# UbiquityRobotics/fiducials

Measured on AMD Instinct MI355X. Metric: frames/sec @1920x1080 20-marker (aruco detect + pose hot path), higher is better.
Workload: dtype u8

## Files before the change

### fiducials_amd/csrc/fid_api.hip

```cpp
#include "fid_kernels.hip"

#include <math.h>
#include <stdio.h>
#include <stdlib.h>
#include <string.h>

#include <new>
#include <string>
#include <vector>

namespace {

enum { ST_GRAY = 0, ST_THRESH, ST_STARTS, ST_PROBE, ST_WALK, ST_APPROX, ST_SORT, ST_NEAR, ST_RESOLVE, ST_IDENT, ST_FILTER, ST_SUBPIX, ST_POSE, ST_SEEDWALK,
       ST_SEEDLESS, ST_COUNT };
const char *const kStageNames[ST_COUNT] = {"to_gray", "threshold", "find_starts", "walk_probe", "walk_full", "approx", "sort_cands",
                                           "near", "resolve", "identify", "filter_markers", "subpix", "pose", "seed_walk", "seedless_chain"};
enum { EV_SEEDWALK0 = 14, EV_SEEDWALK1, EV_SEEDLESS0, EV_SEEDLESS1, EV_POSE0, EV_POSE1, EV_COUNT };
static_assert(EV_SEEDWALK0 > ST_SUBPIX + 1, "the brackets lie behind the stage boundaries");

constexpr int TX = 128, TY = 32, NT = 256;
constexpr int THRW_NT = 512, THRW_WT = 16;
static_assert(THRW_NT * THRW_WT >= 8191, "k_threshold_wide: a row per workgroup");

}

struct fid_ctx;

struct PoseAsk {
    fid_camera cam;
    double len;
    bool cov;
    double sigma;
    fid_map_robust_opts opts;
};

struct PoseRequest {
    enum Kind { MARKER, MAP, MAP_ROBUST };
    Kind kind;
    PoseAsk ask = {};
    bool armed = false;
    bool at_hand = false;
    explicit PoseRequest(Kind k) : kind(k) {}
    inline bool ahead(const fid_ctx *c) const;
    void forget() { at_hand = false; }
    void finished(const fid_ctx *c) { at_hand = ahead(c); }
    bool answers(const PoseAsk &a) const
    {
        return at_hand && !memcmp(&ask.cam, &a.cam, sizeof a.cam) && ask.len == a.len && ask.opts.inlier_px == a.opts.inlier_px &&
               ask.opts.min_markers == a.opts.min_markers && (!a.cov || (ask.cov && ask.sigma == a.sigma));
    }
    void answered(const PoseAsk &a)
    {
        ask = a;
        armed = at_hand = getenv("FID_NO_POSE_AHEAD") == nullptr;
    }
};

struct fid_ctx {
    int device = 0;
    hipStream_t stream = nullptr;
    enum { MAX_SUB = 8 };
    struct Tuning {
        int sub_frames = 0;
        bool sub_shares_set = false;
        int sub_share[MAX_SUB] = {64, 36}, n_sub_share = 2;
        int feed_share[4] = {20, 30, 30, 20};
        int pieces = 0;
        int stagger = 0;
        int fs_barrier = 0;
        int chain_at = 0;
        bool idx_stream = true;
        bool prio = false;
        int thr_xcd = 1;
        int thr_nw = 3, thr_split = 0, thr_rows = 0;
        int seed_shift = 0;
        int seed_kernel = 0;
        bool trace_legacy = false;
        int walk_blocks = 0;
        int walk_blocks_cap = 0;
        int walk2_div = 6;
        int sw_blocks = 0;
        int copy_blocks = 0;
        int probe_refill = 4;
        int probe_refill0 = 0;
        int probe_passes = 1;
        int probe_single = 16;
        int segc_warm = 1;
        int light_x = 1;
        int resolve_lds_kb = 64;
        int resolve_serial = 0;
        int resolve_reg_max = 64;
        int tail_grid = 4096;
        int filter_lds = 256;
    } tune;
    hipStream_t sub_stream[MAX_SUB] = {};
    int sub_prio[MAX_SUB] = {};
    hipStream_t aux_stream[MAX_SUB] = {};
    hipStream_t idx_stream = nullptr;
    hipEvent_t aux_fork[MAX_SUB] = {}, aux_join[MAX_SUB] = {}, aux_idx[MAX_SUB] = {};
    hipEvent_t sub_done[MAX_SUB] = {}, fork_ev = nullptr;
    hipStream_t copy_stream = nullptr;
    hipEvent_t in_ready[MAX_SUB] = {};
    hipEvent_t tail_ev = nullptr, wait_ev = nullptr;
    hipEvent_t wait_copy_ev = nullptr;
    hipEvent_t fs_done[MAX_SUB] = {};
    hipEvent_t walk_done[MAX_SUB] = {};
    hipEvent_t front_done[MAX_SUB] = {};
    hipEvent_t sub_ev[MAX_SUB][EV_COUNT] = {};
    bool blocking = false;
    bool chained = false;
    bool host_feed = false;
    bool from_host_call = false;
    bool piece_chain = false;
    bool tail_recorded = false;
    bool whole_border_walk = false;
    struct Pending {
        const uint8_t *d_src;
        int F, W, H, stride;
        long long fstride;
        fid_encoding enc;
    } pend = {};
    bool in_flight = false;
    bool fed_from_host = false;
    fid_params params;
    fid_limits lim;
    DevParams P;
    std::vector<uint8_t> dict_host;
// ... 106 lines not shown
}

bool refuse_in_flight(fid_ctx *c)
{
    if (c->in_flight) c->last_error = "a submitted batch is in flight: fid_collect first";
    return c->in_flight;
}
bool refuse_no_map(fid_ctx *c)
{
    if (c->map_n == 0) c->last_error = "no map: fid_set_map first";
    return c->map_n == 0;
}
bool refuse_room(fid_ctx *c, int cap_frames)
{
    if (cap_frames < c->last_frames)
        c->last_error = "caller room for " + std::to_string(cap_frames) + " frames, the last call had " + std::to_string(c->last_frames);
    return cap_frames < c->last_frames;
}

int roundup(int v, int m) { return (v + m - 1) / m * m; }

size_t results_bytes(int F, int MM)
{
    auto up = [](size_t v) { return (v + 255) & ~(size_t)255; };
    return up(sizeof(DevGlobal)) + up(sizeof(unsigned) * fid_ctx::MAX_SUB) + up(sizeof(DevCounts) * (size_t)F) + up(sizeof(fid_marker) * (size_t)F * MM) +
           up(sizeof(fid_pose_out) * (size_t)F * MM);
}
void layout_results(fid_ctx *c, int F)
{
    auto up = [](size_t v) { return (v + 255) & ~(size_t)255; };
    const int MM = c->lim.max_markers_per_frame;
    size_t off = 0;
    c->d_global = (DevGlobal *)(c->d_res + off);
    c->h_global = (DevGlobal *)(c->h_res + off);
    off += up(sizeof(DevGlobal));
    c->d_nwork = (unsigned *)(c->d_res + off);
    off += up(sizeof(unsigned) * fid_ctx::MAX_SUB);
    c->d_counts = (DevCounts *)(c->d_res + off);
    c->h_counts = (DevCounts *)(c->h_res + off);
    off += up(sizeof(DevCounts) * (size_t)F);
    c->res_clear_bytes = off;
    c->d_markers = (fid_marker *)(c->d_res + off);
    c->h_markers = (fid_marker *)(c->h_res + off);
    off += up(sizeof(fid_marker) * (size_t)F * MM);
    c->res_markers_end = off;
    c->res_poses_off = off;
    c->d_poses = (fid_pose_out *)(c->d_res + off);
    c->h_poses = (fid_pose_out *)(c->h_res + off);
    off += up(sizeof(fid_pose_out) * (size_t)F * MM);
    c->res_poses_end = off;
}

template <int NW, bool SPLIT>
void launch_thr_stream(dim3 grid, hipStream_t st, const uint8_t *g, long long gfstride, uint32_t *masks, const DevParams &P, int RS, int xcd_map)
{
    using S = ThrStream<3, 4, 13, NW>;
    fid_launch_log("k_threshold_stream", S::NT, S::LDS_BYTES);
    k_threshold_stream<3, 4, 13, NW, SPLIT><<<grid, dim3(S::NT), S::LDS_BYTES, st>>>(g, gfstride, masks, P, RS, xcd_map);
}

fid_status apply_params(fid_ctx *c, const fid_params *p)
{
    if (p->adaptiveThreshWinSizeMin < 3 || p->adaptiveThreshWinSizeMax < p->adaptiveThreshWinSizeMin ||
        p->adaptiveThreshWinSizeStep <= 0)
        return FID_E_INVALID_ARG;
    if (!(p->minMarkerPerimeterRate > 0 && p->maxMarkerPerimeterRate > 0 && p->polygonalApproxAccuracyRate > 0 &&
          p->minCornerDistanceRate >= 0 && p->minDistanceToBorder >= 0 && p->minMarkerDistanceRate >= 0))
        return FID_E_INVALID_ARG;
    if (p->markerBorderBits <= 0) return FID_E_INVALID_ARG;
    int nsc = (p->adaptiveThreshWinSizeMax - p->adaptiveThreshWinSizeMin) / p->adaptiveThreshWinSizeStep + 1;
    if (nsc > FID_MAX_SCALES) return FID_E_UNSUPPORTED;
    DevParams &P = c->P;
    P.nscales = nsc;
    P.rmax = 0;
    for (int i = 0; i < nsc; i++) {
        long long w = p->adaptiveThreshWinSizeMin + (long long)i * p->adaptiveThreshWinSizeStep;
        if (w % 2 == 0) w++;
        if (w > FID_MAX_THR_WIN) {
            c->last_error = "adaptive threshold window " + std::to_string(w) + " px: windows above " + std::to_string(FID_MAX_THR_WIN) +
                            " px (2 x 8191 + 1) are not supported";
            return FID_E_UNSUPPORTED;
        }
        P.win[i] = (int)w;
        if (w / 2 > P.rmax) P.rmax = (int)(w / 2);
    }
    {
        double cdelta = p->adaptiveThreshConstant;
        int i = (int)cdelta;
        P.idelta = i - (i > cdelta);
    }
    P.polyAcc = p->polygonalApproxAccuracyRate;
    P.minCornerDistRate = p->minCornerDistanceRate;
    P.minMarkerDistRate = p->minMarkerDistanceRate;
    P.minDistToBorder = p->minDistanceToBorder;
    P.markerSize = c->dict_ms;
    P.borderBits = p->markerBorderBits;
    P.cellSize = p->perspectiveRemovePixelPerCell;
    P.cellMargin = (int)(p->perspectiveRemoveIgnoredMarginPerCell * p->perspectiveRemovePixelPerCell);
    if (P.markerSize + 2 * P.borderBits > FID_MAX_CELLS) {
        c->last_error = "markerSize + 2 x markerBorderBits = " + std::to_string(P.markerSize + 2 * P.borderBits) + " cells: at most " +
                        std::to_string(FID_MAX_CELLS) + " are supported";
        return FID_E_UNSUPPORTED;
    }
    if (P.cellSize < 1 || P.cellSize - 2 * P.cellMargin < 1) return FID_E_UNSUPPORTED;
    if ((long long)(P.markerSize + 2 * P.borderBits) * P.cellSize > FID_MAX_PATCH) {
        c->last_error = "unwarped patch of (markerSize + 2 x markerBorderBits) x perspectiveRemovePixelPerCell = " +
                        std::to_string((long long)(P.markerSize + 2 * P.borderBits) * P.cellSize) + " px a side: at most " +
                        std::to_string(FID_MAX_PATCH) + " are supported";
        return FID_E_UNSUPPORTED;
    }
    P.minOtsuStdDev = p->minOtsuStdDev;
// ... 210 lines not shown
inline T *frames_from(T *base, int f0, size_t per_frame)
{
    return base ? base + (size_t)f0 * per_frame : nullptr;
}

SubBatch sub_batch_view(fid_ctx *c, const SubPlan &plan, int sb, const uint8_t *d_src, long long fstride, const uint8_t *gray, long long gfstride, int W,
                        int H)
{
    SubBatch s;
    s.sb = sb;
    s.nsub = plan.nsub;
    s.f0 = plan.f0[sb];
    s.Fs = plan.f0[sb + 1] - s.f0;
    s.P = c->P;
    s.P.nframes = s.Fs;
    const DevParams &P = s.P;
    const int f0 = s.f0, lane = c->piece_chain ? (sb & 1) : sb;
    s.st = s.nsub > 1 ? c->sub_stream[lane] : c->stream;
    s.sa = c->aux_stream[lane];
    s.si = (s.nsub == 1 && s.Fs <= 16 && c->idx_stream) ? c->idx_stream : s.sa;
    s.tail = c->piece_chain ? s.sa : s.st;
    s.ev = c->sub_ev[sb];
    const size_t MC = (size_t)P.maxCands, MM = (size_t)P.maxMarkers, MCn = (size_t)P.maxContours, msb = (size_t)(P.markerSize + 2 * P.borderBits);
    s.src = d_src + (long long)f0 * fstride;
    s.gray_dst = c->d_gray + (size_t)f0 * W * H;
    s.g = gray + (long long)f0 * gfstride;
    s.gfstride = gfstride;
    const size_t MS = (size_t)P.maxStarts, chunks = (size_t)P.maxChunks;
    s.masks = frames_from(c->d_masks, f0, (size_t)P.nscales * P.TR * P.TC * MT_ROWS);
    s.starts = frames_from(c->d_starts, f0, MS), s.surv1 = frames_from(c->d_surv1, f0, MS), s.surv = frames_from(c->d_surv, f0, MS);
    s.contours = frames_from(c->d_contours, f0, MCn);
    s.tab = frames_from(c->d_ckpts, f0, 2 * MCn * chunk_tab_pitch(P)), s.pool = frames_from(c->d_pool, f0, chunks * CKW);
    s.counts = c->d_counts + f0;
    s.seedq = frames_from(c->d_seedq, f0, MCn), s.segs = frames_from(c->d_segs, f0, MCn), s.pend = frames_from(c->d_pend, f0, MCn);
    s.seedhash = frames_from(c->d_seedhash, f0, (size_t)P.seedHashCap);
    s.wres = frames_from(c->d_wres, f0, MCn), s.cinfo = frames_from(c->d_cinfo, f0, MCn), s.recs = frames_from(c->d_recs, f0, 2 * MCn);
    s.cbase = frames_from(c->d_cbase, f0, MCn), s.dense = frames_from(c->d_dense, f0, chunks * (CK / 4));
    s.cands = frames_from(c->d_cands, f0, MC), s.sorted = frames_from(c->d_sorted, f0, MC), s.filtered = frames_from(c->d_filtered, f0, MC);
    s.cmeta = frames_from(c->d_cmeta, f0, MC), s.nearb = frames_from(c->d_near, f0, MC * (MC / 32));
    s.worklist = frames_from(c->d_worklist, f0, MC), s.nwork = c->d_nwork + sb;
    s.ident = frames_from(c->d_ident, f0, MC), s.bits = frames_from(c->d_bits, f0, MC * msb * msb);
    s.pre = frames_from(c->d_pre, f0, MM), s.markers = frames_from(c->d_markers, f0, MM), s.filter_scratch = frames_from(c->d_filter_scratch, f0, MC);
    s.accsrc = frames_from(c->d_accsrc, f0, MC), s.mksrc = frames_from(c->d_mksrc, f0, MM);
    s.poses = frames_from(c->d_poses, f0, MM), s.pcov = frames_from(c->d_pcov, f0, MM);
    return s;
}

struct Grids {
    enum Regime { ONE_OR_TWO, FEW, BATCH } regime;
    int gm;
    enum Threshold { THR_STREAM, THR_WIDE, THR_TILES } thr;
    dim3 thr_grid;
    int thr_rows;
    size_t thr_lds;
    unsigned k2blocks;
    bool split_seeds;
    int seed_blocks;
    int wb, wb3, swb, cpb, scb;
    bool single_pass;
    int cap1;
    size_t lds1, lds2;
    int sort_y, light_blocks;
    size_t resolve_lds;
    int near_words;
    int ident_blocks, subpix_blocks;
    size_t ident_lds, filter_lds;
};

Grids launch_grids(const fid_ctx::Tuning &t, const DevParams &P, int Fs)
{
    Grids G;
    const int W = P.W, H = P.H;
    G.regime = Fs <= 2 ? Grids::ONE_OR_TWO : (Fs < 16 ? Grids::FEW : Grids::BATCH);
    const int gm = G.gm = G.regime == Grids::BATCH ? 1 : 16 / Fs;
    bool node_table = P.nscales == 13;
    for (int i = 0; i < P.nscales && node_table; i++) node_table = P.win[i] == 3 + 4 * i;
    G.thr_lds = 0;
    if (node_table) {
        const int cols = 64 * t.thr_nw, strips = (W + cols - 1) / cols;
        int RS = t.thr_rows;
        if (RS <= 0) {
            int segs = (1536 + strips * Fs - 1) / (strips * Fs);
            const int maxsegs = (H + 63) / 64;
            segs = segs < 1 ? 1 : (segs > maxsegs ? maxsegs : segs);
            RS = (H + segs - 1) / segs;
        }
        RS = (RS + 3) & ~3;
        G.thr = Grids::THR_STREAM;
        G.thr_grid = dim3(strips, (H + RS - 1) / RS, Fs);
        G.thr_rows = RS;
    } else if (P.rmax > 40) {
        int bands = (512 + Fs - 1) / Fs;
        const int maxb = (H + 15) / 16;
        bands = bands < 1 ? 1 : (bands > maxb ? maxb : bands);
        const int BH = (H + bands - 1) / bands;
        G.thr = Grids::THR_WIDE;
        G.thr_grid = dim3((H + BH - 1) / BH, 1, Fs);
        G.thr_rows = BH;
        G.thr_lds = (size_t)(W + 1 + THRW_NT / 64) * sizeof(unsigned long long);
    } else {
        int R = P.rmax, RW = TX + 2 * R, RH = TY + 2 * R, PT = (RW + 1) | 1;
        G.thr = Grids::THR_TILES;
        G.thr_grid = dim3((W + TX - 1) / TX, (H + TY - 1) / TY, Fs);
        G.thr_rows = 0;
        G.thr_lds = (size_t)(RH + 1) * PT * sizeof(uint32_t);
    }
    G.split_seeds = t.seed_kernel ? t.seed_kernel == 1 : P.seedShift >= 4;
    {
        long long groups = (long long)P.nscales * P.TR * ((P.WW + 15) / 16);
        long long k2blocks = (groups + 7) / 8;
        if (k2blocks > 256) k2blocks = 256;
        G.k2blocks = (unsigned)k2blocks;
    }
    G.seed_blocks = 0;
    if (G.split_seeds) {
        const SeedUnits su = seed_units(P);
        const int smax = G.regime == Grids::BATCH ? 32 : 512;
        G.seed_blocks = (su.n + 3) / 4 < smax ? (su.n + 3) / 4 : smax;
    }
    int wb = t.walk_blocks > 0 ? t.walk_blocks : (3072 / WALK_WAVES + Fs - 1) / Fs;
    const int wcap = t.walk_blocks_cap > 0 ? t.walk_blocks_cap : (G.regime == Grids::ONE_OR_TWO ? 256 : 64);
    G.wb = wb = wb < 2 ? 2 : (wb > wcap ? wcap : wb);
    const int wb2 = wb > 1 ? wb / 2 : 1;
    G.wb3 = t.walk2_div > 0 ? (wb / t.walk2_div > 0 ? wb / t.walk2_div : 1) : wb2;
    int swb = t.sw_blocks > 0 ? t.sw_blocks : (1024 / SW_WAVES + Fs - 1) / Fs;
    G.swb = swb < 2 ? 2 : (swb > 4 * wcap ? 4 * wcap : swb);
    G.cpb = t.copy_blocks > 0 ? t.copy_blocks : 256;
    G.single_pass = t.probe_passes == 1 && t.probe_refill && gm == 1;
    G.scb = G.regime == Grids::ONE_OR_TWO ? (int)((P.maxContours + 63) / 64 < 4096 ? (P.maxContours + 63) / 64 : 4096) : 32 * gm * t.light_x;
    G.cap1 = pts_cap_first(P);
    G.lds1 = k_approx_lds_bytes(G.cap1);
    G.lds2 = k_approx_lds_bytes(P.maxPerim + 1);
    const size_t MC = (size_t)P.maxCands;
    G.sort_y = (t.light_x > 1 || G.regime != Grids::BATCH) ? 16 : 1;
    G.light_blocks = 32 * gm * t.light_x;
    G.resolve_lds = (size_t)t.resolve_lds_kb * 1024;
    G.near_words = t.resolve_serial ? 0 : (int)((G.resolve_lds - 3 * MC * 4) / 4);
    const int SZ = (P.markerSize + 2 * P.borderBits) * P.cellSize;
    G.ident_blocks = t.tail_grid > 0 ? t.tail_grid : 256 * 4;
    G.ident_lds = (size_t)SZ * SZ;
    G.filter_lds = (size_t)t.filter_lds * sizeof(fid_marker);
    {
        long long items = (long long)Fs * P.maxMarkers * 4;
        const long long bcap = t.tail_grid > 0 ? 4LL * t.tail_grid : 256 * 16;
        G.subpix_blocks = (int)(items < bcap ? items : bcap);
    }
    return G;
}

inline void mark(const fid_ctx *c, const SubBatch &s, hipStream_t st, int idx)
{
    if (c->profile) (void)hipEventRecord(s.ev[idx], st);
}
inline void chain_point(fid_ctx *c, const SubBatch &s, hipStream_t st, int pt)
{
    if (s.sb == s.nsub - 1 && !c->tail_recorded && !c->blocking && c->tune.chain_at <= pt) {
        (void)hipEventRecord(c->tail_ev, st);
        c->tail_recorded = true;
    }
}

fid_status stage_front(fid_ctx *c, const SubBatch &s, const Grids &G, const fid_ctx::Pending &in)
{
    const DevParams &P = s.P;
    const fid_ctx::Tuning &t = c->tune;
    hipStream_t st = s.st;
    const int Fs = s.Fs;
    mark(c, s, st, 0);
    if (in.enc != FID_ENC_MONO8 && (int)in.enc <= FID_ENC_RGBA8)
        hipLaunchKernelGGL(k_to_gray, dim3(2048), dim3(256), 0, st, s.src, in.stride, in.fstride, (int)in.enc, s.gray_dst, P.W, P.H, Fs);
    else if (in.enc != FID_ENC_MONO8)
        hipLaunchKernelGGL(k_raw_to_gray, dim3((P.W + 255) / 256, (P.H + 3) / 4, Fs), dim3(64, 4), 0, st, s.src, in.stride, in.fstride, (int)in.enc,
                           s.gray_dst, P.W, P.H);
    mark(c, s, st, ST_GRAY + 1);
    if (G.thr == Grids::THR_STREAM) {
        if (t.thr_nw == 5 && t.thr_split) launch_thr_stream<5, true>(G.thr_grid, st, s.g, s.gfstride, s.masks, P, G.thr_rows, t.thr_xcd);
        else if (t.thr_nw == 5) launch_thr_stream<5, false>(G.thr_grid, st, s.g, s.gfstride, s.masks, P, G.thr_rows, t.thr_xcd);
        else if (t.thr_split) launch_thr_stream<3, true>(G.thr_grid, st, s.g, s.gfstride, s.masks, P, G.thr_rows, t.thr_xcd);
        else launch_thr_stream<3, false>(G.thr_grid, st, s.g, s.gfstride, s.masks, P, G.thr_rows, t.thr_xcd);
    } else if (G.thr == Grids::THR_WIDE) {
        fid_launch_log("k_threshold_wide", THRW_NT, G.thr_lds);
        hipLaunchKernelGGL((k_threshold_wide<THRW_NT, THRW_WT>), G.thr_grid, dim3(THRW_NT), G.thr_lds, st, s.g, s.gfstride, s.masks, P, G.thr_rows);
    } else {
        hipLaunchKernelGGL((k_threshold<TX, TY, NT>), G.thr_grid, dim3(NT), G.thr_lds, st, s.g, s.gfstride, s.masks, P);
    }
    mark(c, s, st, ST_THRESH + 1);
    if (c->whole_border_walk) return FID_OK;
    if (G.split_seeds) {
        hipLaunchKernelGGL(k_find_starts<false>, dim3(G.k2blocks, Fs), dim3(256), 0, st, s.masks, s.starts, s.counts, c->d_global, (uint2 *)nullptr, P);
        mark(c, s, st, ST_STARTS + 1);
        hipLaunchKernelGGL(k_find_seeds, dim3(G.seed_blocks, Fs), dim3(256), 0, st, s.masks, s.counts, c->d_global, s.seedq, P);
    } else {
        hipLaunchKernelGGL(k_find_starts<true>, dim3(G.k2blocks, Fs), dim3(256), 0, st, s.masks, s.starts, s.counts, c->d_global, s.seedq, P);
        mark(c, s, st, ST_STARTS + 1);
    }
    if (s.nsub > 1) HIPCHK(c, hipEventRecord(c->fs_done[s.sb], st));
    chain_point(c, s, st, 0);
    return FID_OK;
}

fid_status stage_whole_border(fid_ctx *c, const SubBatch &s, const Grids &G)
{
    const DevParams &P = s.P;
    hipStream_t st = s.st;
    const int Fs = s.Fs, gm = G.gm;
    hipLaunchKernelGGL(k_find_starts<false>, dim3(G.k2blocks, Fs), dim3(256), 0, st, s.masks, s.starts, s.counts, c->d_global, (uint2 *)nullptr, P);
    mark(c, s, st, ST_STARTS + 1);
    hipLaunchKernelGGL((k_probe<PROBE0_STEPS, 0>), dim3(64 * gm, Fs), dim3(256), 0, st, s.masks, s.starts, s.surv1, s.counts, c->d_global, P);
    hipLaunchKernelGGL((k_probe<PROBE1_STEPS, 1>), dim3(16 * gm, Fs), dim3(256), 0, st, s.masks, s.surv1, s.surv, s.counts, c->d_global, P);
    mark(c, s, st, ST_PROBE + 1);
    hipLaunchKernelGGL(k_walk_full<0>, dim3(G.wb, Fs), dim3(64 * WALK_WAVES), 0, st, s.masks, s.surv, s.contours, s.tab, s.pool, (DevSegC *)nullptr,
                       (DevPend *)nullptr, s.counts, c->d_global, P);
    mark(c, s, st, ST_WALK + 1);
    fid_launch_log("k_approx", 64, G.lds1);
    hipLaunchKernelGGL(k_approx, dim3(128 * gm, Fs), dim3(64), G.lds1, st, s.contours, s.tab, s.pool, s.cands, s.counts, P, G.cap1, 0,
                       (const uint32_t *)nullptr, (const uint32_t *)nullptr);
    fid_launch_log("k_approx", 64, G.lds2);
    hipLaunchKernelGGL(k_approx, dim3(16 * gm, Fs), dim3(64), G.lds2, st, s.contours, s.tab, s.pool, s.cands, s.counts, P, P.maxPerim + 1, 1,
                       (const uint32_t *)nullptr, (const uint32_t *)nullptr);
    mark(c, s, st, ST_APPROX + 1);
    return FID_OK;
}

fid_status stage_cycle_tracing(fid_ctx *c, const SubBatch &s, const Grids &G)
{
    const DevParams &P = s.P;
    const fid_ctx::Tuning &t = c->tune;
    hipStream_t st = s.st, sa = s.sa, si = s.si;
    const int Fs = s.Fs, gm = G.gm, sb = s.sb;
    const uint4 *probe_tables = (const uint4 *)c->d_probe_tables;
    HIPCHK(c, hipEventRecord(c->aux_fork[sb], st));
    HIPCHK(c, hipStreamWaitEvent(sa, c->aux_fork[sb], 0));
// ... 339 lines not shown
    }
    return rc;
}

fid_status run_detect(fid_ctx *c, const uint8_t *d_src, int F, int W, int H, int stride, long long fstride, fid_encoding enc,
                      fid_marker *out, int cap_per_frame, int *n_per_frame)
{
    if (refuse_in_flight(c) || !out || !n_per_frame || cap_per_frame < 0) {
        c->wait_ev = c->wait_copy_ev = nullptr;
        c->chained = false;
        return FID_E_INVALID_ARG;
    }
    c->blocking = true;
    const fid_status rc = enqueue_detect(c, d_src, F, W, H, stride, fstride, enc);
    c->blocking = false;
    if (rc != FID_OK) {
        c->wait_ev = c->wait_copy_ev = nullptr;
        c->chained = false;
        if (c->last_frames > 0 && !c->in_flight) layout_results(c, c->last_frames);
        return rc;
    }
    return finish_detect(c, out, cap_per_frame, n_per_frame);
}

fid_ctx::Tuning read_tuning()
{
    fid_ctx::Tuning t;
    auto num = [](const char *name, int *v) {
        const char *e = getenv(name);
        if (e) *v = atoi(e);
        return e != nullptr;
    };
    int v = 0;
    num("FID_SUB_FRAMES", &t.sub_frames);
    if (const char *e = getenv("FID_SUB_SHARES")) {
        t.sub_shares_set = true;
        t.n_sub_share = 0;
        for (const char *q = e; *q && t.n_sub_share < fid_ctx::MAX_SUB;) {
            if (atoi(q) > 0) t.sub_share[t.n_sub_share++] = atoi(q);
            while (*q && *q != ',') q++;
            if (*q == ',') q++;
        }
    }
    if (const char *e = getenv("FID_FEED_SHARES")) (void)sscanf(e, "%d,%d,%d,%d", &t.feed_share[0], &t.feed_share[1], &t.feed_share[2], &t.feed_share[3]);
    num("FID_PIECES", &t.pieces);
    num("FID_STAGGER", &t.stagger);
    num("FID_FS_BARRIER", &t.fs_barrier);
    num("FID_CHAIN_AT", &t.chain_at);
    t.idx_stream = getenv("FID_NO_IDX_STREAM") == nullptr;
    if (num("FID_PRIO", &v)) t.prio = v != 0;
    if (num("FID_THR_NW", &v)) t.thr_nw = v == 3 ? 3 : 5;
    if (num("FID_THR_SPLIT", &v)) t.thr_split = v != 0;
    num("FID_THR_ROWS", &t.thr_rows);
    if (num("FID_THR_XCD", &v)) t.thr_xcd = v != 0;
    num("FID_SEED_SHIFT", &t.seed_shift);
    if (const char *e = getenv("FID_SEED_KERNEL")) t.seed_kernel = !strcmp(e, "split") ? 1 : (!strcmp(e, "fused") ? 2 : 0);
    t.trace_legacy = getenv("FID_TRACE") && !strcmp(getenv("FID_TRACE"), "legacy");
    if (num("FID_WALK_BLOCKS", &v) && v > 0) t.walk_blocks = v;
    num("FID_WALK_CAP", &t.walk_blocks_cap);
    num("FID_WALK2_DIV", &t.walk2_div);
    num("FID_SW_BLOCKS", &t.sw_blocks);
    num("FID_COPY_BLOCKS", &t.copy_blocks);
    num("FID_PROBE_REFILL", &t.probe_refill);
    num("FID_PROBE_REFILL0", &t.probe_refill0);
    if (num("FID_PROBE_PASSES", &v) && (v == 1 || v == 2)) t.probe_passes = v;
    if (num("FID_PROBE_SINGLE", &v)) t.probe_single = v < 1 ? 1 : (v > 64 ? 64 : v);
    t.segc_warm = getenv("FID_NO_SEGC_WARM") ? 0 : 1;
    if (num("FID_LIGHT_X", &v)) t.light_x = v > 0 ? v : 1;
    num("FID_RESOLVE_LDS", &t.resolve_lds_kb);
    num("FID_RESOLVE_SERIAL", &t.resolve_serial);
    if (num("FID_RESOLVE_REG_MAX", &v)) t.resolve_reg_max = v < 0 ? 0 : (v > 64 ? 64 : v);
    num("FID_TAIL_GRID", &t.tail_grid);
    if (num("FID_FILTER_LDS", &v)) t.filter_lds = v > 0 ? v : 1;
    return t;
}

}

extern "C" {

void fid_default_params(fid_params *p)
{
    if (!p) return;
    memset(p, 0, sizeof(*p));
    p->adaptiveThreshConstant = 7;
    p->adaptiveThreshWinSizeMin = 3;
    p->adaptiveThreshWinSizeMax = 53;
    p->adaptiveThreshWinSizeStep = 4;
    p->cornerRefinementMethod = 1;
    p->cornerRefinementWinSize = 5;
    p->cornerRefinementMaxIterations = 30;
    p->cornerRefinementMinAccuracy = 0.01;
    p->errorCorrectionRate = 0.6;
    p->minCornerDistanceRate = 0.05;
    p->markerBorderBits = 1;
    p->minDistanceToBorder = 3;
    p->maxErroneousBitsInBorderRate = 0.04;
    p->minMarkerDistanceRate = 0.05;
    p->minMarkerPerimeterRate = 0.1;
    p->maxMarkerPerimeterRate = 4.0;
    p->minOtsuStdDev = 5.0;
    p->perspectiveRemoveIgnoredMarginPerCell = 0.13;
    p->perspectiveRemovePixelPerCell = 8;
    p->polygonalApproxAccuracyRate = 0.01;
}

// ... 27 lines not shown
    if (limits) {
        if (limits->max_width > 0) L.max_width = limits->max_width;
        if (limits->max_height > 0) L.max_height = limits->max_height;
        if (limits->max_batch > 0) L.max_batch = limits->max_batch;
        if (limits->max_starts_per_frame > 0) L.max_starts_per_frame = limits->max_starts_per_frame;
        if (limits->max_contours_per_frame > 0) L.max_contours_per_frame = limits->max_contours_per_frame;
        if (limits->max_candidates_per_frame > 0) L.max_candidates_per_frame = limits->max_candidates_per_frame;
        if (limits->max_markers_per_frame > 0) L.max_markers_per_frame = limits->max_markers_per_frame;
        if (limits->max_points_per_frame > 0) L.max_points_per_frame = limits->max_points_per_frame;
    }
    if (L.max_batch <= 4) {
        if (!limits || limits->max_contours_per_frame <= 0) L.max_contours_per_frame = 65536;
        if (!limits || limits->max_points_per_frame <= 0) L.max_points_per_frame = 16 * 1024 * 1024;
    } else if (L.max_batch <= 16) {
        if (!limits || limits->max_contours_per_frame <= 0) L.max_contours_per_frame = 32768;
        if (!limits || limits->max_points_per_frame <= 0) L.max_points_per_frame = 8 * 1024 * 1024;
    }
    L.max_candidates_per_frame = roundup(L.max_candidates_per_frame, 32);
    if (L.max_candidates_per_frame > 4096 || L.max_batch > 65535 || L.max_markers_per_frame > L.max_candidates_per_frame ||
        L.max_contours_per_frame > (1 << 20)) {
        delete c;
        return FID_E_INVALID_ARG;
    }
    c->lim = L;
    c->dict_ms = dict->marker_size;
    c->dict_maxc = dict->max_correction_bits;
    c->dict_n = dict->n_markers;
    size_t dbytes = (size_t)dict->n_markers * 4 * ((dict->marker_size * dict->marker_size + 7) / 8);
    c->dict_host.assign(dict->bytes, dict->bytes + dbytes);
    c->profile = getenv("FID_PROFILE") && atoi(getenv("FID_PROFILE")) != 0;
    c->tune = read_tuning();
    c->whole_border_walk = c->tune.trace_legacy;
    memset(&c->P, 0, sizeof(c->P));

    fid_status rc = FID_OK;
    auto fail = [&](fid_status s) {
        fid_destroy(c);
        return s;
    };
#define TRY(expr)                         \
    do {                                  \
        rc = (expr);                      \
        if (rc != FID_OK) return fail(rc); \
    } while (0)
#define TRYHIP(expr)                                   \
    do {                                               \
        hipError_t e_ = (expr);                        \
        if (e_ != hipSuccess) {                        \
            fprintf(stderr, "fid_create: %s: %s\n", #expr, hipGetErrorString(e_)); \
            return fail(e_ == hipErrorOutOfMemory ? FID_E_OUT_OF_MEMORY : FID_E_HIP); \
        }                                              \
    } while (0)
    TRYHIP(hipSetDevice(device));
    TRYHIP(hipStreamCreateWithFlags(&c->stream, hipStreamNonBlocking));
    for (hipEvent_t &e : c->pose_ev) TRYHIP(hipEventCreate(&e));
    TRYHIP(hipEventCreateWithFlags(&c->fork_ev, hipEventDisableTiming));
    TRYHIP(hipEventCreateWithFlags(&c->tail_ev, hipEventDisableTiming));
    int prio_lo = 0, prio_hi = 0;
    (void)hipDeviceGetStreamPriorityRange(&prio_lo, &prio_hi);
    for (int sb = 0; sb < fid_ctx::MAX_SUB; sb++) {
        int prio = c->tune.prio ? prio_hi + sb : prio_lo;
        if (prio > prio_lo) prio = prio_lo;
        c->sub_prio[sb] = prio;
        TRYHIP(hipEventCreateWithFlags(&c->aux_fork[sb], hipEventDisableTiming));
        TRYHIP(hipEventCreateWithFlags(&c->aux_join[sb], hipEventDisableTiming));
        TRYHIP(hipEventCreateWithFlags(&c->sub_done[sb], hipEventDisableTiming));
        TRYHIP(hipEventCreateWithFlags(&c->walk_done[sb], hipEventDisableTiming));
        TRYHIP(hipEventCreateWithFlags(&c->in_ready[sb], hipEventDisableTiming));
        TRYHIP(hipEventCreateWithFlags(&c->fs_done[sb], hipEventDisableTiming));
        TRYHIP(hipEventCreateWithFlags(&c->front_done[sb], hipEventDisableTiming));
        TRYHIP(hipEventCreateWithFlags(&c->aux_idx[sb], hipEventDisableTiming));
        for (hipEvent_t &e : c->sub_ev[sb]) TRYHIP(hipEventCreate(&e));
    }
    const size_t F = L.max_batch, MC = L.max_candidates_per_frame, MM = L.max_markers_per_frame;
    TRY(dalloc(c, &c->d_subpix_mask, (size_t)(2 * SP_MAXWIN_MAX + 1) * (2 * SP_MAXWIN_MAX + 1)));
    TRY(dalloc(c, &c->d_probe_tables, (size_t)4096));
    hipLaunchKernelGGL(k_probe_tables, dim3(1), dim3(256), 0, nullptr, c->d_probe_tables);
    TRYHIP(hipGetLastError());
    TRYHIP(hipDeviceSynchronize());
    TRY(dalloc(c, &c->d_dict, dbytes));
    TRYHIP(hipMemcpy(c->d_dict, c->dict_host.data(), dbytes, hipMemcpyHostToDevice));
    rc = apply_params(c, params);
    if (rc != FID_OK) return fail(rc);
    TRY(dalloc(c, &c->d_gray, F * L.max_width * L.max_height));
    c->masks_bytes = masks_elems(c, L.max_width, L.max_height, (int)F) * sizeof(uint32_t);
    c->masks_bytes += (size_t)F * c->P.nscales * (L.max_height + 2) * 16 * sizeof(uint32_t);
    TRYHIP(hipMalloc((void **)&c->d_masks, c->masks_bytes));
    TRY(dalloc(c, &c->d_starts, F * L.max_starts_per_frame));
    TRY(dalloc(c, &c->d_surv1, F * L.max_starts_per_frame));
    TRY(dalloc(c, &c->d_surv, F * L.max_starts_per_frame));
    c->max_chunks = (L.max_points_per_frame + CK - 1) / CK;
    TRY(dalloc(c, &c->d_pool, F * (size_t)c->max_chunks * CKW));
    if (!c->whole_border_walk) {
        TRY(dalloc(c, &c->d_segs, F * L.max_contours_per_frame));
        TRY(dalloc(c, &c->d_pend, F * L.max_contours_per_frame));
        TRY(dalloc(c, &c->d_seedq, F * L.max_contours_per_frame));
        c->seed_hash_cap = 1;
        while (c->seed_hash_cap < 2 * L.max_contours_per_frame) c->seed_hash_cap *= 2;
        TRY(dalloc(c, &c->d_seedhash, F * (size_t)c->seed_hash_cap));
        TRYHIP(hipMemset(c->d_seedhash, 0, F * (size_t)c->seed_hash_cap * sizeof(unsigned long long)));
        TRY(dalloc(c, &c->d_wres, F * L.max_contours_per_frame));
        TRY(dalloc(c, &c->d_cinfo, F * L.max_contours_per_frame));
        TRY(dalloc(c, &c->d_cbase, F * L.max_contours_per_frame));
        TRY(dalloc(c, &c->d_recs, 2 * F * L.max_contours_per_frame));
        TRY(dalloc(c, &c->d_dense, F * (size_t)c->max_chunks * (CK / 4) + 2));
    }
// ... 733 lines not shown
```

### fiducials_amd/csrc/fid_kernels.hip

```cpp
#include <hip/hip_runtime.h>
#include <stdint.h>
#include <float.h>
#include <limits.h>

#include <type_traits>
#include <utility>

#include "fid_device.h"
#include "../../include/fid_abi.h"

#define WAVE 64

__device__ __forceinline__ int lane_id() { return threadIdx.x & (WAVE - 1); }

__device__ __forceinline__ unsigned long long ballot64(int pred) { return __ballot(pred); }

#define FID_DPP(OLD, V, CTRL, RMASK) __builtin_amdgcn_update_dpp((OLD), (V), (CTRL), (RMASK), 0xf, false)
#define FID_DPP_SCAN_STEPS(STEP) STEP(0x111, 0xf) STEP(0x112, 0xf) STEP(0x114, 0xf) STEP(0x118, 0xf) STEP(0x142, 0xa) STEP(0x143, 0xc)

__device__ __forceinline__ int wave_iscan(int v)
{
#define S_(C, M) v += FID_DPP(0, v, C, M);
    FID_DPP_SCAN_STEPS(S_)
#undef S_
// ... 435 lines not shown
{
    const uint32_t lo = (uint32_t)b, hi = (uint32_t)(b >> 32);
    asm("s_mov_b32 m0, %2\n\tv_writelane_b32 %0, %3, m0\n\tv_writelane_b32 %1, %4, m0"
                 : "+v"(a0), "+v"(a1)
                 : "s"(sel), "s"(lo), "s"(hi));
}

__device__ __forceinline__ void park_quad(uint32_t &a0, uint32_t &a1, unsigned long long b0, unsigned long long b1, unsigned long long b2,
                                          unsigned long long b3, int sel)
{
#ifdef FID_PARK_WRITELANE
    park_pair(a0, a1, b0, sel);
    park_pair(a0, a1, b1, sel + 1);
    park_pair(a0, a1, b2, sel + 2);
    park_pair(a0, a1, b3, sel + 3);
#else
    unsigned long long keep;
    asm("s_mov_b64 %2, exec\n\t"
        "s_lshl_b64 exec, 1, %3\n\t"
        "v_mov_b32 %0, %4\n\tv_mov_b32 %1, %5\n\t"
        "s_lshl_b64 exec, exec, 1\n\t"
        "v_mov_b32 %0, %6\n\tv_mov_b32 %1, %7\n\t"
        "s_lshl_b64 exec, exec, 1\n\t"
        "v_mov_b32 %0, %8\n\tv_mov_b32 %1, %9\n\t"
        "s_lshl_b64 exec, exec, 1\n\t"
        "v_mov_b32 %0, %10\n\tv_mov_b32 %1, %11\n\t"
        "s_mov_b64 exec, %2"
        : "+v"(a0), "+v"(a1), "=&s"(keep)
        : "s"(sel), "s"((uint32_t)b0), "s"((uint32_t)(b0 >> 32)), "s"((uint32_t)b1), "s"((uint32_t)(b1 >> 32)), "s"((uint32_t)b2),
          "s"((uint32_t)(b2 >> 32)), "s"((uint32_t)b3), "s"((uint32_t)(b3 >> 32))
        : "scc");
#endif
}

__device__ __forceinline__ void park_quad64(unsigned long long &a, unsigned long long b0, unsigned long long b1, unsigned long long b2,
                                            unsigned long long b3, int sel)
{
    unsigned long long keep;
    asm("s_mov_b64 %1, exec\n\t"
        "s_lshl_b64 exec, 1, %2\n\t"
        "v_mov_b64 %0, %3\n\t"
        "s_lshl_b64 exec, exec, 1\n\t"
        "v_mov_b64 %0, %4\n\t"
        "s_lshl_b64 exec, exec, 1\n\t"
        "v_mov_b64 %0, %5\n\t"
        "s_lshl_b64 exec, exec, 1\n\t"
        "v_mov_b64 %0, %6\n\t"
        "s_mov_b64 exec, %1"
        : "+v"(a), "=&s"(keep)
        : "s"(sel), "s"(b0), "s"(b1), "s"(b2), "s"(b3)
        : "scc");
}

template <int WMIN, int WSTEP, int NS, int NW, bool SPLIT>
__global__ __launch_bounds__(64 * (NW + 1)) void k_threshold_stream(const uint8_t *__restrict__ gray, long long gfstride,
                                                                      uint32_t *__restrict__ masks, const DevParams P, int RS, int xcd_map)
{
    using C = ThrStream<WMIN, WSTEP, NS, NW>;
    constexpr int R = C::R, PADL = C::PADL, RAWW = C::RAWW, NCHUNK = C::NCHUNK, ROWPAD = C::ROWPAD, LEAD = C::LEAD;
    extern __shared__ __attribute__((aligned(16))) uint2 thr_ring[];
    const int lane = threadIdx.x & 63;
    const int wid = __builtin_amdgcn_readfirstlane(threadIdx.x >> 6);
    unsigned bx = blockIdx.x, by = blockIdx.y, bz = blockIdx.z;
    if (xcd_map) {
        const unsigned gx = gridDim.x, gy = gridDim.y, N = gx * gy * gridDim.z;
        const unsigned L = bx + gx * (by + gy * bz), j = L & 7u, k = L >> 3, q = N >> 3, r = N & 7u;
        const unsigned T = j * q + (j < r ? j : r) + k;
        bx = T % gx;
        const unsigned t2 = T / gx;
        by = t2 % gy;
        bz = t2 / gy;
    }
    const int xs = (int)bx * C::COLS, ys = (int)by * RS, f = (int)bz;
    const int W = P.W, H = P.H, gs = P.gstride;
    const uint8_t *g = gray + (long long)f * gfstride;
    const int yend = ys + RS < H ? ys + RS : H;
    const int nsteps = (yend - ys + 3) >> 2;
    const int Q0 = (ys >> 2) + ROWPAD / 4;

    struct RawQuad {
        uint32_t v01[NCHUNK], v23[NCHUNK];
    };
    auto load_quad = [&](int Q, RawQuad &q) {
        const int yb = 4 * Q - ROWPAD;
        const uint8_t *rp[4];
#pragma unroll
        for (int i = 0; i < 4; i++) {
            int y = yb + i;
            y = y < 0 ? 0 : (y >= H ? H - 1 : y);
            rp[i] = g + (long long)y * gs;
        }
#pragma unroll
        for (int c = 0; c < NCHUNK; c++) {
            int x = xs - PADL + 64 * c + lane;
            x = x < 0 ? 0 : (x >= W ? W - 1 : x);
            q.v01[c] = (uint32_t)rp[0][x] | ((uint32_t)rp[1][x] << 16);
            q.v23[c] = (uint32_t)rp[2][x] | ((uint32_t)rp[3][x] << 16);
        }
    };
    auto store_quad = [&](int Q, const RawQuad &q) {
        uint2 *dst = thr_ring + (Q & (C::DEPTH - 1)) * RAWW;
        uint32_t c01 = 0, c23 = 0;
#pragma unroll
        for (int c = 0; c < NCHUNK; c++) {
            const uint32_t s01 = wave_iscan_dpp(q.v01[c]), s23 = wave_iscan_dpp(q.v23[c]);
            const int j = 64 * c + lane;
            if (j < RAWW) dst[j] = make_uint2(pk_add16(s01, c01), pk_add16(s23, c23));
            c01 = pk_add16(c01, (uint32_t)__builtin_amdgcn_readlane((int)s01, 63));
            c23 = pk_add16(c23, (uint32_t)__builtin_amdgcn_readlane((int)s23, 63));
        }
    };
    for (int q = Q0 - LEAD + wid; q <= Q0 + LEAD; q += NW + 1) {
        RawQuad rq;
        load_quad(q, rq);
        store_quad(q, rq);
    }
    __syncthreads();

    if (wid == NW) {
        const int last = Q0 + nsteps - 1 + LEAD;
        RawQuad cur, nxt;
        if (Q0 + LEAD + 1 <= last) load_quad(Q0 + LEAD + 1, cur);
        for (int k = 0; k < nsteps; k++) {
            const int Q = Q0 + k + LEAD + 1;
            if (Q + 1 <= last) load_quad(Q + 1, nxt);
            if (Q <= last) store_quad(Q, cur);
            __syncthreads();
            cur = nxt;
        }
        return;
    }

    const int colw = 64 * wid;
    const bool wave_on = xs + colw < W;
    const unsigned long long vmask = ballot64(xs + colw + lane < W);
    const uint32_t jb = (uint32_t)(colw + lane);
    int zoff = 0;
    if (SPLIT) asm volatile("" : "+s"(zoff));
    auto slot_base = [&](int Q) { return thr_ring + (Q & (C::DEPTH - 1)) * RAWW + jb; };
    auto hquad = [&](int Q, int r) {
        const uint2 *b = slot_base(Q);
        const uint2 hi = b[PADL + r], lo = (b + zoff)[PADL - r - 1];
        return make_uint2(pk_sub16(hi.x, lo.x), pk_sub16(hi.y, lo.y));
    };
    int V[NS];
    uint32_t ca[NS], cb[NS], cc[NS];
#ifndef FID_PARK_MOV32
    unsigned long long acc[NS];
#else
    uint32_t acc0[NS], acc1[NS];
#endif
    if (wave_on) {
        static_for<NS>([&](auto sc) {
            constexpr int s = decltype(sc)::value;
            constexpr int r = (WMIN + s * WSTEP) / 2, w2 = (2 * r + 1) * (2 * r + 1);
            const uint16_t *ring16 = reinterpret_cast<const uint16_t *>(thr_ring);
            uint32_t sum = 0;
            for (int rho = ys - 1 - r + ROWPAD; rho <= ys - 1 + r + ROWPAD; rho++) {
                const int e = (((rho >> 2) & (C::DEPTH - 1)) * RAWW + (int)jb) * 4 + (rho & 3);
                sum += (uint16_t)(ring16[e + (PADL + r) * 4] - ring16[e + (PADL - r - 1) * 4]);
            }
            V[s] = (int)sum - (P.idelta * w2 - (w2 - 1) / 2);
#ifndef FID_PARK_MOV32
            acc[s] = 0ull;
#else
            acc0[s] = acc1[s] = 0;
#endif
            if constexpr ((r & 3) == 1) {
                const uint2 e = hquad(Q0 + (r + 3) / 4 - 1, r);
                ca[s] = e.x;
                cb[s] = e.y;
                cc[s] = hquad(Q0 - (r - 1) / 4 - 1, r).y;
            } else {
                ca[s] = hquad(Q0 + (r + 1) / 4 - 1, r).y;
                cb[s] = cc[s] = 0;
            }
        });
    }
    const long long plane = (long long)P.TR * P.TC * MT_ROWS;
    uint32_t *mframe = masks + (long long)f * NS * plane;
    auto flush = [&](int yblk) {
        const int yrow = yblk + lane;
        if (yrow < yend) {
            const int wc = (xs + colw) >> 5;
            uint32_t *q = mframe + mask_word(P.TC, yrow + 1, MASK_PADW + wc);
            const bool two = xs + colw + 32 < W;
            const uint32_t m0w = (uint32_t)vmask, m1w = (uint32_t)(vmask >> 32);
#pragma unroll
            for (int s = 0; s < NS; s++) {
#ifndef FID_PARK_MOV32
                q[(long long)s * plane] = (uint32_t)acc[s] & m0w;
                if (two) q[(long long)s * plane + MT_ROWS] = (uint32_t)(acc[s] >> 32) & m1w;
#else
                q[(long long)s * plane] = acc0[s] & m0w;
                if (two) q[(long long)s * plane + MT_ROWS] = acc1[s] & m1w;
#endif
            }
        }
    };
    for (int k = 0; k < nsteps; k++) {
        if (wave_on) {
            const int qo = Q0 + k;
            const int sel = (4 * k) & 63;
            uint32_t g0, g1, g2, g3;
            {
                const uint2 *b = slot_base(qo);
                const uint2 hi = b[PADL], lo = b[PADL - 1];
                const uint32_t a = pk_sub16(hi.x, lo.x), c = pk_sub16(hi.y, lo.y);
                g0 = a & 0xffffu;
                g1 = a >> 16;
                g2 = c & 0xffffu;
                g3 = c >> 16;
            }
            struct Rd {
                uint2 eh, el, lh, ll;
            };
            auto fetch = [&](auto sc) {
                constexpr int s = decltype(sc)::value;
                constexpr int r = (WMIN + s * WSTEP) / 2;
                Rd q;
                constexpr int de = (r & 3) == 1 ? (r + 3) / 4 : (r + 1) / 4, dl = (r & 3) == 1 ? (r - 1) / 4 : (r + 1) / 4;
                const uint2 *be = slot_base(qo + de), *bl = slot_base(qo - dl);
                q.eh = be[PADL + r];
                q.el = (be + zoff)[PADL - r - 1];
                q.lh = bl[PADL + r];
                q.ll = (bl + zoff)[PADL - r - 1];
                return q;
            };
            Rd cur = fetch(std::integral_constant<int, 0>{});
            static_for<NS>([&](auto sc) {
                constexpr int s = decltype(sc)::value;
                constexpr int r = (WMIN + s * WSTEP) / 2, w2 = (2 * r + 1) * (2 * r + 1);
                Rd nxt = cur;
                if constexpr (s + 1 < NS) nxt = fetch(std::integral_constant<int, s + 1>{});
                __builtin_amdgcn_sched_barrier(0);
                const uint2 e = make_uint2(pk_sub16(cur.eh.x, cur.el.x), pk_sub16(cur.eh.y, cur.el.y));
                const uint2 l = make_uint2(pk_sub16(cur.lh.x, cur.ll.x), pk_sub16(cur.lh.y, cur.ll.y));
                uint32_t elo, ehi, llo, lhi;
                if constexpr ((r & 3) == 1) {
                    elo = __builtin_amdgcn_alignbit(cb[s], ca[s], 16);
                    ehi = __builtin_amdgcn_alignbit(e.x, cb[s], 16);
                    llo = cc[s];
                    lhi = l.x;
                    ca[s] = e.x;
                    cb[s] = e.y;
                    cc[s] = l.y;
                } else {
                    elo = __builtin_amdgcn_alignbit(e.x, ca[s], 16);
                    ehi = __builtin_amdgcn_alignbit(e.y, e.x, 16);
                    llo = l.x;
                    lhi = l.y;
                    ca[s] = e.y;
                }
                const thr_s16x2 dlo = __builtin_bit_cast(thr_s16x2, pk_sub16(elo, llo));
                const thr_s16x2 dhi = __builtin_bit_cast(thr_s16x2, pk_sub16(ehi, lhi));
                const thr_s16x2 first = {1, 0}, second = {0, 1};
                int v = V[s];
                v = __builtin_amdgcn_sdot2(dlo, first, v, false);
                const unsigned long long b0 = ballot64(v >= __mul24((int)g0, w2));
                v = __builtin_amdgcn_sdot2(dlo, second, v, false);
                const unsigned long long b1 = ballot64(v >= __mul24((int)g1, w2));
                v = __builtin_amdgcn_sdot2(dhi, first, v, false);
                const unsigned long long b2 = ballot64(v >= __mul24((int)g2, w2));
                v = __builtin_amdgcn_sdot2(dhi, second, v, false);
                const unsigned long long b3 = ballot64(v >= __mul24((int)g3, w2));
                V[s] = v;
#ifndef FID_PARK_MOV32
                park_quad64(acc[s], b0, b1, b2, b3, sel);
#else
                park_quad(acc0[s], acc1[s], b0, b1, b2, b3, sel);
#endif
                cur = nxt;
            });
            if (sel == 60 || k == nsteps - 1) flush(ys + ((4 * k) & ~63));
        }
        __syncthreads();
    }
}

__device__ __forceinline__ unsigned long long seedhash_key(uint32_t state, int scale) { return (unsigned long long)state | ((unsigned long long)scale << 29); }
__device__ __forceinline__ unsigned seedhash_slot(unsigned long long key, int cap)
{
    return (unsigned)((key * 0x9E3779B97F4A7C15ull) >> 40) & (unsigned)(cap - 1);
}
__device__ __forceinline__ void seedhash_insert(unsigned long long *__restrict__ tab, int cap, int gen, unsigned long long key, unsigned idx)
{
    const unsigned long long ent = ((unsigned long long)gen << 54) | (key << 20) | idx;
    unsigned h = seedhash_slot(key, cap);
    unsigned long long old = tab[h];
    for (;;) {
        if ((int)(old >> 54) != gen) {
            const unsigned long long prev = atomicCAS(&tab[h], old, ent);
            if (prev == old) return;
            old = prev;
            continue;
        }
        h = (h + 1) & (unsigned)(cap - 1);
        old = tab[h];
    }
}
__device__ __forceinline__ unsigned seedhash_find(const unsigned long long *__restrict__ tab, int cap, int gen, unsigned long long key)
{
    unsigned h = seedhash_slot(key, cap);
    for (int probes = 0; probes < cap; probes++) {
        const unsigned long long e = tab[h];
        if ((int)(e >> 54) != gen) return SEG_INVALID;
        if (((e >> 20) & 0x3ffffffffull) == key) return (unsigned)(e & 0xfffffu);
        h = (h + 1) & (unsigned)(cap - 1);
    }
    return SEG_INVALID;
}

__device__ __forceinline__ uint32_t fill_toward_msb_rev(uint32_t rseed, uint32_t rruns)
{
    const uint32_t t = rruns + rseed;
    return (t & rseed) | (~t & rruns);
}
__device__ __forceinline__ uint32_t fill_toward_lsb(uint32_t seed, uint32_t runs)
{
    const uint32_t m = __brev(runs);
    return __brev(fill_toward_msb_rev(__brev(seed) & m, m));
}
__device__ __forceinline__ uint32_t low_run_has_seed(uint32_t seed, uint32_t runs)
{
    const uint32_t low = runs & ~(runs + 1u);
    return (low & seed) != 0u ? 1u : 0u;
}

__device__ __forceinline__ void divmod_small(unsigned a, unsigned b, float rcp_b, unsigned &q, unsigned &r)
// ... 3985 lines not shown
```

Baseline: 41600.

## Flatten threshold-stream grid and balance row pieces across occupancy slots

Reworks the threshold-stream kernel launch into a 1D grid. Each block walks a contiguous range of quarter-row units that can span strips and frames, and the per-piece body is factored into a device function. The default segment count is now derived from measured occupancy (blocks per CU times CU count) instead of a fixed constant. Optional env knobs allow an even-share split meant to balance tail work across slots. The change adds per-block division and loop overhead and moves some params into scalar registers.

After: 41350. No clear change (-0.6%).

```diff
diff --git a/fiducials_amd/csrc/fid_api.hip b/fiducials_amd/csrc/fid_api.hip
--- a/fiducials_amd/csrc/fid_api.hip
+++ b/fiducials_amd/csrc/fid_api.hip
@@ -73,6 +73,8 @@
         bool prio = false;
         int thr_xcd = 1;
         int thr_nw = 3, thr_split = 0, thr_rows = 0;
+        int thr_shares = 0, thr_rounds = 0;
+        int thr_slots = 0;
         int seed_shift = 0;
         int seed_kernel = 0;
         bool trace_legacy = false;
@@ -285,11 +287,18 @@
 }
 
 template <int NW, bool SPLIT>
-void launch_thr_stream(dim3 grid, hipStream_t st, const uint8_t *g, long long gfstride, uint32_t *masks, const DevParams &P, int RS, int xcd_map)
+void launch_thr_stream(dim3 grid, hipStream_t st, const uint8_t *g, long long gfstride, uint32_t *masks, const DevParams &P, const ThrCut &cut, int xcd_map)
 {
     using S = ThrStream<3, 4, 13, NW>;
     fid_launch_log("k_threshold_stream", S::NT, S::LDS_BYTES);
-    k_threshold_stream<3, 4, 13, NW, SPLIT><<<grid, dim3(S::NT), S::LDS_BYTES, st>>>(g, gfstride, masks, P, RS, xcd_map);
+    k_threshold_stream<3, 4, 13, NW, SPLIT><<<grid, dim3(S::NT), S::LDS_BYTES, st>>>(g, gfstride, masks, P, cut, xcd_map);
+}
+
+template <int NW, bool SPLIT>
+hipError_t thr_stream_per_cu(int *n)
+{
+    using S = ThrStream<3, 4, 13, NW>;
+    return hipOccupancyMaxActiveBlocksPerMultiprocessor(n, k_threshold_stream<3, 4, 13, NW, SPLIT>, S::NT, S::LDS_BYTES);
 }
 
 fid_status apply_params(fid_ctx *c, const fid_params *p)
@@ -606,6 +615,7 @@
     enum Threshold { THR_STREAM, THR_WIDE, THR_TILES } thr;
     dim3 thr_grid;
     int thr_rows;
+    ThrCut thr_cut;
     size_t thr_lds;
     unsigned k2blocks;
     bool split_seeds;
@@ -632,17 +642,35 @@
     G.thr_lds = 0;
     if (node_table) {
         const int cols = 64 * t.thr_nw, strips = (W + cols - 1) / cols;
-        int RS = t.thr_rows;
-        if (RS <= 0) {
-            int segs = (1536 + strips * Fs - 1) / (strips * Fs);
-            const int maxsegs = (H + 63) / 64;
-            segs = segs < 1 ? 1 : (segs > maxsegs ? maxsegs : segs);
-            RS = (H + segs - 1) / segs;
-        }
-        RS = (RS + 3) & ~3;
+        const long long pairs = (long long)strips * Fs, hq = (H + 3) / 4, pieces = pairs * (H >= 128 ? H / 64 : 1);
+        ThrCut &cut = G.thr_cut;
+        cut = ThrCut{(unsigned)strips, 0u, 0u, 0u, 0u};
+        long long n = 0;
+        if (t.thr_rows <= 0) {
+            const long long rounds = pieces / t.thr_slots < t.thr_rounds ? pieces / t.thr_slots : t.thr_rounds;
+            n = t.thr_shares > 0 ? t.thr_shares : rounds * t.thr_slots;
+            if (n > pieces) n = pieces;
+        }
+        if (n > 0) {
+            cut.base = (unsigned)(pairs * hq / n);
+            cut.rem = (unsigned)(pairs * hq % n);
+        } else {
+            int RS = t.thr_rows;
+            if (RS <= 0) {
+                const long long want = 3LL * t.thr_slots / 2;
+                long long segs = (want + pairs - 1) / pairs;
+                const int maxsegs = (H + 63) / 64;
+                segs = segs < 1 ? 1 : (segs > maxsegs ? maxsegs : segs);
+                RS = (int)((H + segs - 1) / segs);
+            }
+            RS = (RS + 3) & ~3;
+            cut.segq = (unsigned)(RS / 4);
+            cut.segs = (unsigned)((hq + cut.segq - 1) / cut.segq);
+            n = pairs * cut.segs;
+        }
         G.thr = Grids::THR_STREAM;
-        G.thr_grid = dim3(strips, (H + RS - 1) / RS, Fs);
-        G.thr_rows = RS;
+        G.thr_grid = dim3((unsigned)n, 1, 1);
+        G.thr_rows = 0;
     } else if (P.rmax > 40) {
         int bands = (512 + Fs - 1) / Fs;
         const int maxb = (H + 15) / 16;
@@ -728,10 +756,10 @@
                            s.gray_dst, P.W, P.H);
     mark(c, s, st, ST_GRAY + 1);
     if (G.thr == Grids::THR_STREAM) {
-        if (t.thr_nw == 5 && t.thr_split) launch_thr_stream<5, true>(G.thr_grid, st, s.g, s.gfstride, s.masks, P, G.thr_rows, t.thr_xcd);
-        else if (t.thr_nw == 5) launch_thr_stream<5, false>(G.thr_grid, st, s.g, s.gfstride, s.masks, P, G.thr_rows, t.thr_xcd);
-        else if (t.thr_split) launch_thr_stream<3, true>(G.thr_grid, st, s.g, s.gfstride, s.masks, P, G.thr_rows, t.thr_xcd);
-        else launch_thr_stream<3, false>(G.thr_grid, st, s.g, s.gfstride, s.masks, P, G.thr_rows, t.thr_xcd);
+        if (t.thr_nw == 5 && t.thr_split) launch_thr_stream<5, true>(G.thr_grid, st, s.g, s.gfstride, s.masks, P, G.thr_cut, t.thr_xcd);
+        else if (t.thr_nw == 5) launch_thr_stream<5, false>(G.thr_grid, st, s.g, s.gfstride, s.masks, P, G.thr_cut, t.thr_xcd);
+        else if (t.thr_split) launch_thr_stream<3, true>(G.thr_grid, st, s.g, s.gfstride, s.masks, P, G.thr_cut, t.thr_xcd);
+        else launch_thr_stream<3, false>(G.thr_grid, st, s.g, s.gfstride, s.masks, P, G.thr_cut, t.thr_xcd);
     } else if (G.thr == Grids::THR_WIDE) {
         fid_launch_log("k_threshold_wide", THRW_NT, G.thr_lds);
         hipLaunchKernelGGL((k_threshold_wide<THRW_NT, THRW_WT>), G.thr_grid, dim3(THRW_NT), G.thr_lds, st, s.g, s.gfstride, s.masks, P, G.thr_rows);
@@ -1177,6 +1205,8 @@
     if (num("FID_THR_NW", &v)) t.thr_nw = v == 3 ? 3 : 5;
     if (num("FID_THR_SPLIT", &v)) t.thr_split = v != 0;
     num("FID_THR_ROWS", &t.thr_rows);
+    num("FID_THR_SHARES", &t.thr_shares);
+    if (num("FID_THR_ROUNDS", &v) && v > 0) t.thr_rounds = v;
     if (num("FID_THR_XCD", &v)) t.thr_xcd = v != 0;
     num("FID_SEED_SHIFT", &t.seed_shift);
     if (const char *e = getenv("FID_SEED_KERNEL")) t.seed_kernel = !strcmp(e, "split") ? 1 : (!strcmp(e, "fused") ? 2 : 0);
@@ -1310,6 +1340,15 @@
         }                                              \
     } while (0)
     TRYHIP(hipSetDevice(device));
+    {
+        int per_cu = 0, cus = 0;
+        const fid_ctx::Tuning &t = c->tune;
+        TRYHIP(t.thr_nw == 5 ? (t.thr_split ? thr_stream_per_cu<5, true>(&per_cu) : thr_stream_per_cu<5, false>(&per_cu))
+                             : (t.thr_split ? thr_stream_per_cu<3, true>(&per_cu) : thr_stream_per_cu<3, false>(&per_cu)));
+        TRYHIP(hipDeviceGetAttribute(&cus, hipDeviceAttributeMultiprocessorCount, device));
+        if (per_cu < 1 || cus < 1) return fail(FID_E_HIP);
+        c->tune.thr_slots = per_cu * cus;
+    }
     TRYHIP(hipStreamCreateWithFlags(&c->stream, hipStreamNonBlocking));
     for (hipEvent_t &e : c->pose_ev) TRYHIP(hipEventCreate(&e));
     TRYHIP(hipEventCreateWithFlags(&c->fork_ev, hipEventDisableTiming));
diff --git a/fiducials_amd/csrc/fid_kernels.hip b/fiducials_amd/csrc/fid_kernels.hip
--- a/fiducials_amd/csrc/fid_kernels.hip
+++ b/fiducials_amd/csrc/fid_kernels.hip
@@ -511,29 +511,23 @@
         : "scc");
 }
 
+__device__ __forceinline__ int lane_id_here()
+{
+    int lane;
+    asm volatile("v_mbcnt_lo_u32_b32 %0, -1, 0\n\tv_mbcnt_hi_u32_b32 %0, -1, %0" : "=v"(lane));
+    return lane;
+}
+
 template <int WMIN, int WSTEP, int NS, int NW, bool SPLIT>
-__global__ __launch_bounds__(64 * (NW + 1)) void k_threshold_stream(const uint8_t *__restrict__ gray, long long gfstride,
-                                                                      uint32_t *__restrict__ masks, const DevParams P, int RS, int xcd_map)
+__device__ __forceinline__ void thr_stream_piece(const uint8_t *__restrict__ g, uint32_t *__restrict__ mframe, const DevParams &P, int xs, int ys,
+                                                 int yend, int wid)
 {
     using C = ThrStream<WMIN, WSTEP, NS, NW>;
     constexpr int R = C::R, PADL = C::PADL, RAWW = C::RAWW, NCHUNK = C::NCHUNK, ROWPAD = C::ROWPAD, LEAD = C::LEAD;
     extern __shared__ __attribute__((aligned(16))) uint2 thr_ring[];
-    const int lane = threadIdx.x & 63;
-    const int wid = __builtin_amdgcn_readfirstlane(threadIdx.x >> 6);
-    unsigned bx = blockIdx.x, by = blockIdx.y, bz = blockIdx.z;
-    if (xcd_map) {
-        const unsigned gx = gridDim.x, gy = gridDim.y, N = gx * gy * gridDim.z;
-        const unsigned L = bx + gx * (by + gy * bz), j = L & 7u, k = L >> 3, q = N >> 3, r = N & 7u;
-        const unsigned T = j * q + (j < r ? j : r) + k;
-        bx = T % gx;
-        const unsigned t2 = T / gx;
-        by = t2 % gy;
-        bz = t2 / gy;
-    }
-    const int xs = (int)bx * C::COLS, ys = (int)by * RS, f = (int)bz;
-    const int W = P.W, H = P.H, gs = P.gstride;
-    const uint8_t *g = gray + (long long)f * gfstride;
-    const int yend = ys + RS < H ? ys + RS : H;
+    const int lane = lane_id_here();
+    int W = P.W, H = P.H, gs = P.gstride, idelta = P.idelta, TC = P.TC;
+    asm volatile("" : "+s"(W), "+s"(H), "+s"(gs), "+s"(idelta), "+s"(TC));
     const int nsteps = (yend - ys + 3) >> 2;
     const int Q0 = (ys >> 2) + ROWPAD / 4;
 
@@ -619,7 +613,7 @@
                 const int e = (((rho >> 2) & (C::DEPTH - 1)) * RAWW + (int)jb) * 4 + (rho & 3);
                 sum += (uint16_t)(ring16[e + (PADL + r) * 4] - ring16[e + (PADL - r - 1) * 4]);
             }
-            V[s] = (int)sum - (P.idelta * w2 - (w2 - 1) / 2);
+            V[s] = (int)sum - (idelta * w2 - (w2 - 1) / 2);
 #ifndef FID_PARK_MOV32
             acc[s] = 0ull;
 #else
@@ -636,13 +630,12 @@
             }
         });
     }
-    const long long plane = (long long)P.TR * P.TC * MT_ROWS;
-    uint32_t *mframe = masks + (long long)f * NS * plane;
+    const long long plane = (long long)P.TR * TC * MT_ROWS;
     auto flush = [&](int yblk) {
-        const int yrow = yblk + lane;
+        const int yrow = yblk + lane_id_here();
         if (yrow < yend) {
             const int wc = (xs + colw) >> 5;
-            uint32_t *q = mframe + mask_word(P.TC, yrow + 1, MASK_PADW + wc);
+            uint32_t *q = mframe + mask_word(TC, yrow + 1, MASK_PADW + wc);
             const bool two = xs + colw + 32 < W;
             const uint32_t m0w = (uint32_t)vmask, m1w = (uint32_t)(vmask >> 32);
 #pragma unroll
@@ -734,6 +727,50 @@
             if (sel == 60 || k == nsteps - 1) flush(ys + ((4 * k) & ~63));
         }
         __syncthreads();
+    }
+}
+
+struct ThrCut {
+    unsigned strips, segq, segs, base, rem;
+};
+
+template <int WMIN, int WSTEP, int NS, int NW, bool SPLIT>
+__global__ __launch_bounds__(64 * (NW + 1)) void k_threshold_stream(const uint8_t *__restrict__ gray, long long gfstride,
+                                                                      uint32_t *__restrict__ masks, const DevParams P, const ThrCut cut, int xcd_map)
+{
+    using C = ThrStream<WMIN, WSTEP, NS, NW>;
+    const int wid = __builtin_amdgcn_readfirstlane(threadIdx.x >> 6);
+    unsigned T = blockIdx.x;
+    if (xcd_map) {
+        const unsigned N = gridDim.x, j = T & 7u, k = T >> 3, q = N >> 3, r = N & 7u;
+        T = j * q + (j < r ? j : r) + k;
+    }
+    auto udiv_s = [](unsigned a, unsigned b) { return (unsigned)__builtin_amdgcn_readfirstlane((int)(a / b)); };
+    const unsigned Hq = (unsigned)(P.H + 3) >> 2;
+    unsigned qa, qz;
+    if (cut.segq) {
+        const unsigned t2 = udiv_s(T, cut.strips), strip = T - t2 * cut.strips, fr = udiv_s(t2, cut.segs), sg = t2 - fr * cut.segs;
+        const unsigned top = (fr * cut.strips + strip) * Hq;
+        qa = top + sg * cut.segq;
+        qz = qa + cut.segq < top + Hq ? qa + cut.segq : top + Hq;
+    } else {
+        qa = T * cut.base + (T < cut.rem ? T : cut.rem);
+        qz = qa + cut.base + (T < cut.rem ? 1u : 0u);
+    }
+    const long long plane = (long long)P.TR * P.TC * MT_ROWS;
+    const unsigned pair = udiv_s(qa, Hq);
+    unsigned yq = qa - pair * Hq, f = udiv_s(pair, cut.strips), strip = pair - f * cut.strips;
+    while (qa < qz) {
+        const unsigned npq = qz - qa < Hq - yq ? qz - qa : Hq - yq;
+        const int ys = (int)yq * 4, yend = ys + 4 * (int)npq < P.H ? ys + 4 * (int)npq : P.H;
+        thr_stream_piece<WMIN, WSTEP, NS, NW, SPLIT>(gray + (long long)f * gfstride, masks + (long long)f * NS * plane, P,
+                                                     (int)strip * C::COLS, ys, yend, wid);
+        qa += npq;
+        yq = 0;
+        if (++strip == cut.strips) {
+            strip = 0;
+            f++;
+        }
     }
 }
 
```
